# bab2min/Kiwi

Measured on AMD Instinct MI355X. Metric: sentences/sec on batched analyze(), device kernels with inputs resident in HBM (dictionary scan + lattice + Viterbi/Knlm, top-1); host-to-host rate: see e2e, higher is better.
Workload: dtype int32+f32; 1 GPU; c2-64k: 65536 synthetic sentences ({'exact_jamo': 40}), synthetic 'full' model (kiwi_amd/synth.py), Knlm, top-1; sentences_per_gpu=65536, chunks_per_gpu=65536, jamo_per_gpu=2621440, parallelism=shard1, device_bytes=9402884427, rerun_chunks=0

## Files before the change

### kiwi_amd/csrc/engine.hip

```cpp
#include <hip/hip_runtime.h>
#include <unistd.h>
#include <cstdio>
#include <cstring>
#include <ctime>
#include <algorithm>
#include <atomic>
#include <cstdlib>
#include <chrono>
#include <condition_variable>
#include <functional>
#include <map>
#include <mutex>
#include <numeric>
#include <stdexcept>
#include <thread>
#include "engine.hpp"
#include "pretok.hpp"
#include "hostpool.hpp"
#include "post_fast.hpp"
#include "viterbi_kernel.hpp"
#include "exact_math.hpp"
#include "cong_global.hpp"
#include "chr_freq.hpp"
#include "typo_lattice_kernel.hpp"
#include "typo_graph_kernel.hpp"
#include "cong_query_kernel.hpp"

namespace kamd
{
	__global__ void k_dict_scan(ModelView M, BatchView B, WorkView W, uint32_t chunkBegin, uint32_t chunkCount);
	template<int GW> __global__ void k_build_lattice(ModelView M, BatchView B, WorkView W, SearchParams P, const uint32_t* chunkList, uint32_t chunkCount, uint32_t ldsBytes);
	__global__ void k_build_lattice_big(ModelView M, BatchView B, WorkView W, SearchParams P, uint32_t chunkBegin, uint32_t chunkCount, uint32_t ldsBytes, uint32_t waveLayout);
	__global__ void k_lattice_wave(ModelView M, BatchView B, WorkView W, SearchParams P, const uint32_t* chunkList, uint32_t chunkCount, uint32_t ldsBytes, uint32_t matchRatio16, uint32_t expandMode);
	__global__ void k_expand_cands(ModelView M, BatchView B, WorkView W, uint32_t chunkBegin, uint32_t chunkCount, uint32_t transposedOrder, const uint8_t* distMask);
	__global__ void k_expand_pos(ModelView M, BatchView B, WorkView W, SearchParams P, uint32_t chunkBegin, uint32_t chunkCount, const float* nodeTypoAll, uint32_t useChr);
	__global__ void k_unk_chr(ModelView M, BatchView B, WorkView W, ChrView C, uint32_t chunkBegin, uint32_t chunkCount, uint32_t hiTok, uint32_t loTok);
	__global__ void k_unk_chr_freq(ModelView M, BatchView B, WorkView W, ChrView C, ChrFreqParams Q, float chrBias, uint32_t chunkBegin, uint32_t chunkCount, uint32_t hiTok, uint32_t loTok);

	namespace
	{
		void hipCheck(hipError_t e, const char* what)
		{
			if (e != hipSuccess) throw std::runtime_error{ std::string{ "HIP error in " } + what + ": " + hipGetErrorString(e) };
		}
#define HIPCHECK(x) hipCheck((x), #x)

		struct DevBlockCache
		{
			struct Block { void* p; size_t cap; int device; };
			std::mutex mu; std::vector<Block> blocks; size_t bytes = 0;
			static constexpr size_t kMaxBlocks = 256, kMaxBytes = 64ull << 30;
			static void release(const Block& b) { if (b.device < 0) (void)hipHostFree(b.p); else (void)hipFree(b.p); }
			void* take(size_t n, size_t& capOut, int device)
			{
				std::lock_guard<std::mutex> g{ mu };
				size_t best = blocks.size();
				for (size_t i = 0; i < blocks.size(); ++i)
					if (blocks[i].device == device && blocks[i].cap >= n && blocks[i].cap <= 2 * n + (1u << 20) && (best == blocks.size() || blocks[i].cap < blocks[best].cap)) best = i;
				if (best == blocks.size()) return nullptr;
// ... 258 lines not shown
		impl->device = device;
		HIPCHECK(hipSetDevice(device));
		HIPCHECK(hipStreamCreateWithFlags(&impl->stream, hipStreamNonBlocking));
		HIPCHECK(hipStreamCreateWithFlags(&impl->stream2, hipStreamNonBlocking));
		for (auto& ls : impl->latStream) HIPCHECK(hipStreamCreateWithFlags(&ls, hipStreamNonBlocking));
		{
			int least = 0, greatest = 0;
			const bool plain = [] { const char* e = std::getenv("KAMD_COPY_PRIORITY"); return !(e && std::atoi(e) == 1); }();
			if (plain || hipDeviceGetStreamPriorityRange(&least, &greatest) != hipSuccess || least == greatest) HIPCHECK(hipStreamCreateWithFlags(&impl->streamCopy, hipStreamNonBlocking));
			else HIPCHECK(hipStreamCreateWithPriority(&impl->streamCopy, hipStreamNonBlocking, greatest));
		}
		HIPCHECK(hipEventCreateWithFlags(&impl->lastDone, hipEventDisableTiming)); HIPCHECK(hipEventCreateWithFlags(&impl->joinEv, hipEventDisableTiming));
		HIPCHECK(hipEventCreate(&impl->latFork)); for (auto& ev : impl->latJoin) HIPCHECK(hipEventCreate(&ev));

		if (const char* sb = std::getenv("KAMD_SUBBATCHES")) impl->subBatches = std::atoi(sb);
		const FlatModel& m = impl->model;
		ModelView& v = impl->dview;
		v.h = m.h;
		using I_ = Engine::Impl;
		v.forms = impl->up(m.forms, I_::kTempForms); v.formChars = impl->up(m.formChars, I_::kTempChars); v.formCand = impl->up(m.formCand, I_::kTempCand);
		{
			std::vector<MorphRec> dm = m.morphs;
			for (size_t i = 0; i < dm.size(); ++i) { dm[i].feat = (uint16_t)m.morphPath[i]; dm[i].prevFlags = (uint8_t)(m.morphPath[i] >> 16); }
			v.morphs = impl->up(dm, I_::kTempMorphs);
			std::vector<CandStatic> unk(2);
			for (int k = 0; k < 2; ++k)
			{
				const uint32_t mid = (k == 0 ? T_NNG : T_NNP) + 1u;
				std::memcpy(&unk[k].m0, &dm[mid], 32);
				const uint32_t firstWid = (dm[mid].flags & MF_SINGLE) ? dm[mid].lmId : m.chunkLm[dm[mid].chunkOff];
				unk[k].x = Quad{ mid, firstWid, 0, 0 };
			}
			v.unkPacks = impl->up(unk);
		}
		v.chunkMorph = impl->up(m.chunkMorph, I_::kTempChunks); v.chunkLm = impl->up(m.chunkLm, I_::kTempChunks); v.chunkPos = impl->up(m.chunkPos, 2 * I_::kTempChunks);
		v.sbInfo = impl->up(m.sbInfo, I_::kTempMorphs); v.morphPath = impl->up(m.morphPath, I_::kTempMorphs);
		v.trie = impl->up(m.trie); v.trieKeys = impl->up(m.trieKeys); v.trieChild = impl->up(m.trieChild); v.trieRoot = impl->up(m.trieRoot);
		v.trieEdges = impl->up(m.trieEdges); v.trieEdgeMask = m.trieEdgeMask;
		v.lmNodes = impl->up(m.lmNodes); v.lmKeys = impl->up(m.lmKeys); v.lmValues = impl->up(m.lmValues); v.lmRoot = impl->up(m.lmRoot);
		if (m.congDim)
		{
			v.lmHash = impl->up(m.congHash); v.lmHashMask = m.congHashMask; v.lmRoot2 = impl->up(m.congRoot2); v.lmBackoff = impl->up(m.congBackoff);
			v.h.bosNode = 0;
			impl->cong = CongDev{ impl->up(m.congCtxEmb), impl->up(m.congOutEmb), m.congDim, m.congDim + 8, m.congVlTMax, m.congVlBits };
			impl->hasCong = true;
			if (impl->wantCongGlobal)
			{
				if (!m.congWindow) throw std::runtime_error{ "Cannot open ConG model with distant tokens: the file has no window sections" };
				if (m.congWindow != 7) throw std::runtime_error{ "kiwi_amd: CoNgram window size must be 7 (the reference instantiates CoNgramState<7> only)" };
				CongGDev& g = impl->congG;
				g.ctxConf = impl->up(m.congCtxConf); g.distEmb = impl->up(m.congDistEmb); g.distConf = impl->up(m.congDistConf); g.posConf = impl->up(m.congPosConf);
				g.distMask = impl->up(m.congDistMask); g.window = m.congWindow; g.keyBytes = m.congKeyBytes; g.hist = nullptr; g.itemScratch = nullptr;
				impl->hasCongG = true;
			}
		}
		else { v.lmHash = impl->up(m.lmHash); v.lmHashMask = m.lmHashMask; v.lmRoot2 = impl->up(m.lmRoot2); v.lmBackoff = impl->up(m.lmBackoff); }
		v.lmHtxNode = (m.congDim || m.lmHtxNode.empty()) ? nullptr : impl->up(m.lmHtxNode);
		v.formDialect = nullptr;
		v.morphDialect = m.morphDialect.empty() ? nullptr : impl->up(m.morphDialect, I_::kTempMorphs);
		if (v.morphDialect) HIPCHECK(hipMemset(const_cast<uint16_t*>(v.morphDialect) + m.morphDialect.size(), 0, 2 * I_::kTempMorphs));
		v.formUnkChr = nullptr; v.formChrTok = nullptr;
		v.lmChain = nullptr;
		if (!m.congDim && !m.lmBackoff.empty())
		{
			std::vector<uint32_t> chain(2 * m.lmBackoff.size());
			for (size_t n = 0; n < m.lmBackoff.size(); ++n)
// ... 525 lines not shown
			b.order = order;
			b.subBatches = S;
			if (b.typo.typo)
			{
				b.typoOrder.resize(nC);
				std::iota(b.typoOrder.begin(), b.typoOrder.end(), 0u);
				for (uint32_t k = 0; k < S; ++k)
				{
					const uint32_t c0 = (uint32_t)((uint64_t)nC * k / S), c1 = (uint32_t)((uint64_t)nC * (k + 1) / S);
					std::stable_sort(b.typoOrder.begin() + c0, b.typoOrder.begin() + c1, [&](uint32_t a, uint32_t c) { return b.typoNeed[a] > b.typoNeed[c]; });
				}
				upload(b.dTypoOrder, b.typoOrder, I.streamCopy);
			}
			HIPCHECK(hipStreamSynchronize(I.streamCopy));
		}
		const size_t nEv = 6 * (size_t)S + 2;
		while (I.evs.size() < nEv) { hipEvent_t e; HIPCHECK(hipEventCreate(&e)); I.evs.push_back(e); }
		if (I.haveLast) HIPCHECK(hipStreamWaitEvent(sA, I.lastDone, 0));
		if (b.pretok && b.pretok->hasTemps())
		{
			const TempOverlay& o = b.pretok->overlay; const FlatModel& m = I.model; const ModelView& v = I.dview;
			using I_ = Engine::Impl;
			if (o.forms.size() > I_::kTempForms || o.morphs.size() > I_::kTempMorphs || o.formChars.size() > I_::kTempChars || o.formCand.size() > I_::kTempCand || o.chunkMorph.size() > I_::kTempChunks)
				throw std::invalid_argument{ "kiwi_amd: too many temporary forms / morphemes in the pretokenized spans of one call" };
			auto put = [&](const auto* devBase, size_t at, const auto& vec)
			{
				using T = std::remove_cv_t<std::remove_pointer_t<decltype(devBase)>>;
				if (!vec.empty()) HIPCHECK(hipMemcpyAsync(const_cast<T*>(devBase) + at, vec.data(), vec.size() * sizeof(T), hipMemcpyHostToDevice, sA));
			};
			put(v.forms, o.nBaseForms, o.forms); put(v.formChars, m.formChars.size() - 1, o.formChars); put(v.formCand, m.formCand.size(), o.formCand);
			put(v.morphs, o.nBaseMorphs, b.pretok->devMorphs); put(v.chunkMorph, m.chunkMorph.size(), o.chunkMorph); put(v.chunkLm, m.chunkLm.size(), o.chunkLm);
			put(v.chunkPos, m.chunkPos.size(), o.chunkPos); put(v.sbInfo, o.nBaseMorphs, o.sbInfo); put(v.morphPath, o.nBaseMorphs, o.morphPath);
			if (v.formUnkChr) { put(v.formUnkChr, o.nBaseForms, o.formUnkChr); put(v.formChrTok, m.formChars.size() - 1, o.formChrTok); }
		}
		HIPCHECK(hipMemsetAsync(b.dResults.p, 0, nC * sizeof(DevChunkResult), sA));
		HIPCHECK(hipMemsetAsync(b.dOutCounters.p, 0, 128, sA));
		HIPCHECK(hipMemcpyAsync(b.dStateAt.p, b.wv.stateBase, (size_t)nC * 8, hipMemcpyDeviceToDevice, sA));
		if (b.slotCap) HIPCHECK(hipMemsetAsync(b.dSlotTable.p, 0, (size_t)I.histSlots() * 16, sA));
		HIPCHECK(hipMemsetAsync(I.counter.p, 0, 256, sA));
		HIPCHECK(hipMemsetAsync(b.dNNodes.p, 0, (size_t)nC * 4, sA));
		HIPCHECK(hipMemsetAsync(b.dExpanded.p, 0, nC, sA));
		if (getenv("KAMD_HANGDUMP")) HIPCHECK(hipMemsetAsync(b.dNodeStCnt.p, 0xFF, (size_t)b.nodeBase[nC] * 4, sA));
		const bool variant64 = I.histStates() ? !(I.groupLanesForced && I.groupLanes == 16) : (I.groupLanesForced && I.groupLanes == 64);
		const uint32_t nGroups = (I.histStates() || b.typo.typo || I.hasCong) ? (variant64 ? 1u : 4u)
			: 64u / (uint32_t)(I.groupLanesForced ? I.groupLanes : 8);
		const uint32_t maxWork = (nC + S - 1) / S + 1;
		const uint32_t persistBlocks = I.histStates() ? I.persistBlocks / 12 * I.histBlocksPerCu() : I.persistBlocks;
		const uint32_t maxBlocks = std::min(persistBlocks, (maxWork + nGroups - 1) / nGroups);
		const size_t groupScratchBytes = I.hasSbg ? sizeof(GroupScratchT<BIGQ_SBG>) : I.hasCongG ? sizeof(GroupScratchCong<BIGQ_SBG>) : I.hasCong ? sizeof(GroupScratchCong<BIGQ>) : sizeof(GroupScratch);
		I.bigScratch.ensure((size_t)maxBlocks * nGroups * groupScratchBytes * std::min(S, 2u));
		b.wv.bigScratch = I.bigScratch.as<uint8_t>(); b.wv.bigScratchBytes = (uint32_t)groupScratchBytes;
		if (I.histStates())
		{
			const void* before = I.sbgScratch.p;
			I.sbgScratch.ensure((size_t)maxBlocks * nGroups * sizeof(SbgScratch) * std::min(S, 2u));
			if (I.sbgScratch.p != before) HIPCHECK(hipMemsetAsync(I.sbgScratch.p, 0, I.sbgScratch.cap, sA));
		}
		const uint32_t ldsBytes = searchKernelLdsBytes(I.groupLanes);
		if (!b.typo.typo)
		{
			const bool wave = I.latticeWave && I.latticeGroupForced == 0;
			const uint32_t ratioKey = wave ? (I.latticeRatio16 & 0x3FFFu) : 0x10000u;
			const uint32_t budget = b.pretok ? 0u : wave ? I.latticeWaveBudget : I.latticeLdsBudget;
			const uint32_t classesKey = ratioKey * 31u + budget / 16u;
			if (b.latClassesKey != classesKey || b.latClasses.size() != S)
			{
// ... 1491 lines not shown
```

### kiwi_amd/csrc/flat_model.hpp

```cpp
#pragma once
#include <cstdint>
#include <cmath>
#include <string>
#include <vector>
#include "kchars.hpp"

namespace kamd
{
	enum FormFlag : uint8_t
	{
		FF_ZCODA_APPENDABLE = 1, FF_ZSIOT_APPENDABLE = 2, FF_HAS_JCLASS = 4, FF_HAS_ANY_FULL = 8,
		FF_FIRST_IS_CODA = 16,
		FF_IS_STAG = 32,
		FF_STARTS_WITH_A = 64,
		FF_ENDS_WITH_SSC = 128,
	};
	struct FormRec
	{
		uint32_t candOff;
		uint32_t charOff;
		uint16_t candCnt;
		uint8_t len;
		uint8_t numSpaces;
		uint8_t flags;
// ... 49 lines not shown
	struct TrieEdgeSlot { uint32_t node, key, child; int32_t value; };
	static_assert(sizeof(TrieEdgeSlot) == 16, "TrieEdgeSlot");
	constexpr uint32_t TRIE_EDGE_EMPTY = 0xFFFFFFFFu;
	KAMD_HD uint32_t trieEdgeHash(uint32_t node, uint32_t key) { uint32_t h = node * 0x9E3779B1u + key * 0x85EBCA6Bu; h ^= h >> 15; h *= 0x2C1B3C6Du; h ^= h >> 13; return h; }
	constexpr int32_t TRIE_NONE = -1, TRIE_SUBMATCH = -2;
	constexpr uint16_t LF_STR_SSC = 1u << 13, LF_PREV_ZSIOT = 1u << 14, LF_TAG_SSC = 1u << 15;

	struct LmSlot { uint32_t node, wid; int32_t value; float ll; };
	static_assert(sizeof(LmSlot) == 16, "LmSlot");
	constexpr uint32_t LM_SLOT_EMPTY = 0xFFFFFFFFu;
	struct LmRootRec { int32_t value; float ll; };
	struct LmBackoff { int32_t lower; float gamma; };
	KAMD_HD uint32_t lmHashOf(uint32_t node, uint32_t wid) { uint32_t h = node * 0x9E3779B1u ^ (wid * 0x85EBCA77u); h ^= h >> 15; h *= 0x2C1B3C6Du; h ^= h >> 13; return h; }

	struct LmNodeRec
	{
		uint32_t nextOff, numNexts;
		int32_t lower;
		float ll, gamma;
	};
	static_assert(sizeof(LmNodeRec) == 20, "LmNodeRec");

	struct ModelHeader
	{
		uint32_t nForms, nMorphs, vocabSize, nTrieNodes, nTrieEdges, nLmNodes, nLmEdges;
		int32_t bosNode;
		float unkLl;
		uint32_t specialMorph[6];
		uint32_t maxFormLen;
		uint32_t lmOrder;
		uint32_t lmKeyBytes;
	};

	struct ModelView
	{
		ModelHeader h;
		const FormRec* forms;
		const uint16_t* formChars;
		const uint32_t* formCand;
		const MorphRec* morphs;
		const uint32_t* chunkMorph;
		const uint32_t* chunkLm;
		const uint8_t* chunkPos;
		const uint8_t* sbInfo;
		const uint32_t* morphPath;
		const TrieNodeRec* trie;
		const uint16_t* trieKeys;
		const uint32_t* trieChild;
		const uint32_t* trieRoot;
		const LmNodeRec* lmNodes;
		const uint32_t* lmKeys;
		const int32_t* lmValues;
		const int32_t* lmRoot;
		const LmSlot* lmHash; uint32_t lmHashMask;
		const LmRootRec* lmRoot2;
		const LmBackoff* lmBackoff;
		const void* unkPacks;
		const int32_t* lmHtxNode;
		const float* formUnkChr;
		const uint16_t* formChrTok;
		const uint16_t* formDialect; const uint16_t* morphDialect;
		const uint32_t* lmChain;
		const TrieEdgeSlot* trieEdges; uint32_t trieEdgeMask;
	};

	struct SbgView
	{
		uint32_t vocabSize = 0, windowSize = 0;
		const uint32_t* ptrs = nullptr;
		const uint32_t* keys = nullptr;
		const float* comps = nullptr;
		const float* discnts = nullptr;
		const uint8_t* valid = nullptr;
		float logWindowSize = 0;
		bool present() const { return vocabSize != 0; }
	};

	struct CongNodeRec { uint32_t nextOff, numNexts; int32_t lower; uint32_t value; };
	struct CongView
	{
		uint32_t dim = 0, stride = 0, nCtx = 0, vocabSize = 0;
		const uint8_t* ctxEmb = nullptr; const uint8_t* outEmb = nullptr;
		const CongNodeRec* nodes = nullptr; const uint32_t* keys = nullptr; const int32_t* values = nullptr; const int32_t* root = nullptr;
		uint32_t rootSize = 0;
		uint32_t vlTMax = 0xFFFFFFFFu, vlBits = 0;
		uint32_t window = 0;
		uint32_t keyBytes = 4;
		const float* ctxConf = nullptr;
		const uint8_t* distEmb = nullptr;
		const float* distConf = nullptr;
// ... 276 lines not shown
```

### kiwi_amd/csrc/lattice_expand.hpp

```cpp
#pragma once
#include <hip/hip_runtime.h>
#include "device_types.hpp"
#include "feature.hpp"

namespace kamd
{
	__device__ __forceinline__ float leftBoundaryScore(uint32_t t)
	{
		if (t == 2 * T_MAX) return 5.f;
		if (t < T_MAX) return (t == T_NNP || t == T_NP || t == T_IC) ? -1.f : (t == T_SB ? -3.f : 0.f);
		const uint8_t r = (uint8_t)(t - T_MAX);
		return (isEClass(r) || isJClass(r) || isSuffixTag(r) || r == T_VCP) ? -1.f : 0.f;
	}
	__device__ __forceinline__ uint32_t posCandKind(const SearchParams& P, uint32_t flags, uint8_t tag, bool spaceBefore)
	{
		if (P.splitComplex && (flags & MF_HAS_COMPLEX)) return 0;
		if (tag == T_Z_CODA || tag == T_Z_SIOT) return (tag == T_Z_SIOT && !(P.splitSaisiot || P.mergeSaisiot)) ? 0u : 2u;
		if (!(flags & MF_SINGLE) && (flags & MF_HA_CONTRACTION) && spaceBefore) return 0;
		return 1;
	}

	__device__ __forceinline__ CandStatic candStaticOf(const ModelView& M, uint32_t mid)
	{
		const uint4* mr = reinterpret_cast<const uint4*>(M.morphs + mid);
		CandStatic o; const uint4 r0 = mr[0], r1 = mr[1];
		o.m0 = Quad{ r0.x, r0.y, r0.z, r0.w }; o.m1 = Quad{ r1.x, r1.y, r1.z, r1.w };
		const uint32_t flags = o.m1.y & 0xFFFF; const uint8_t tag = (uint8_t)o.m1.z;
		const uint32_t firstWid = (flags & MF_SINGLE) ? o.m0.x : M.chunkLm[o.m0.z];
		const uint32_t sbType = tag == T_SB ? M.sbInfo[mid] : 0;
		const uint32_t secondWid = (!(flags & MF_SINGLE) && (o.m1.w & 0xFF) >= 2) ? M.chunkLm[o.m0.z + 1] : 0;
		o.x = Quad{ mid, firstWid, sbType, secondWid };
		return o;
	}
	__device__ __forceinline__ uint32_t candClassOf(uint32_t tag, uint32_t socket, uint32_t flags)
	{
		if (tag == T_Z_CODA) return 0;
		if (tag == T_Z_SIOT) return 1;
		if (!socket) return 2;
		return (flags & MF_SINGLE) ? 3 : 4;
	}
}
```

### kiwi_amd/csrc/lattice_kernels.hip

```cpp
#include <hip/hip_runtime.h>
#include "device_types.hpp"
#include "feature.hpp"
#include "lattice_connect.hpp"
#include "lattice_expand.hpp"
#include "chr_freq.hpp"

namespace kamd
{
	__device__ __forceinline__ uint32_t trieChild(const ModelView& M, uint32_t node, uint16_t c, int32_t& value)
	{
		if (node == 0) { const uint32_t ch = M.trieRoot[c]; value = ch ? M.trie[ch].value : TRIE_NONE; return ch; }
		uint32_t h = trieEdgeHash(node, c) & M.trieEdgeMask;
		for (;;)
		{
			const uint4 s = reinterpret_cast<const uint4*>(M.trieEdges)[h];
			if (s.x == node && s.y == (uint32_t)c) { value = (int32_t)s.w; return s.z; }
			if (s.x == TRIE_EDGE_EMPTY) { value = TRIE_NONE; return 0; }
			h = (h + 1) & M.trieEdgeMask;
		}
	}

	__global__ void __launch_bounds__(256) k_dict_scan(ModelView M, BatchView B, WorkView W, uint32_t chunkBegin, uint32_t chunkCount)
	{
		const uint32_t lane = threadIdx.x & 63;
// ... 719 lines not shown
		DevNode* fin = W.nodes + nBase;
		const uint32_t textOff = B.textOffset[chunk];
		for (uint32_t idx = 0; idx < G; ++idx) latticeEmitNode(M, L, str, cls, queue, fin, idx, n, nConn, textOff);
		{
			uint32_t packTop = 0;
			const uint32_t packCap = W.packBase[chunk + 1] - W.packBase[chunk];
			for (uint32_t i = 0; i < nConn; ++i) { fin[i].packOff = packTop; packTop += fin[i].candCnt; }
			if (packTop > packCap) { W.results[chunk].status = CS_ERR_NODE_OVERFLOW; return; }
		}
		W.nNodes[chunk] = nConn;
		if (nConn <= 2) W.results[chunk].status = CS_NO_LATTICE;
	}

	__global__ void __launch_bounds__(64) k_expand_cands(ModelView M, BatchView B, WorkView W, uint32_t chunkBegin, uint32_t chunkCount, uint32_t transposedOrder, const uint8_t* distMask)
	{
		if (blockIdx.x >= chunkCount) return;
		const uint32_t chunk = chunkBegin + blockIdx.x;
		if (W.results[chunk].status != CS_OK || W.expanded[chunk]) return;
		const uint32_t nBase = W.nodeBase[chunk], G = W.nNodes[chunk];
		CandStatic* packs = W.packs + W.packBase[chunk];
		const uint32_t* blk = W.blockBits;
		auto blocked = [&](uint32_t m2) -> bool { return blk && ((blk[m2 >> 5] >> (m2 & 31)) & 1); };
		for (uint32_t i = 1 + threadIdx.x; i + 1 < G; i += blockDim.x)
		{
			const DevNode nd = W.nodes[nBase + i];
			if (nd.form == NOFORM) continue;
			const uint32_t candOff = M.forms[nd.form].candOff;
			uint32_t kept = 0;
			for (uint32_t k = 0; k < nd.candCnt; ++k)
			{
				const uint32_t mid = M.formCand[candOff + k];
				if (blocked(mid)) continue;
				++kept;
				const CandStatic o = candStaticOf(M, mid);
				uint32_t at = 0;
				if (transposedOrder)
				{
					auto cls = [&](uint32_t m2) -> uint32_t
					{
						const MorphRec r = M.morphs[m2];
						uint32_t c2 = 2u * candClassOf(r.tag, r.socket, r.flags);
						if (distMask && c2 == 4u) { const uint32_t fw = (r.flags & MF_SINGLE) ? r.lmId : M.chunkLm[r.chunkOff]; c2 += (distMask[fw >> 3] >> (fw & 7)) & 1u; }
						return c2;
					};
					const uint32_t mine = cls(mid);
					for (uint32_t j = 0; j < nd.candCnt; ++j)
					{
						if (j == k) continue;
						const uint32_t mj = M.formCand[candOff + j];
						if (blocked(mj)) continue;
						const uint32_t other = cls(mj);
						if (other < mine || (other == mine && j < k)) ++at;
					}
				}
				else if (blk) { for (uint32_t j = 0; j < k; ++j) if (!blocked(M.formCand[candOff + j])) ++at; }
				else at = k;
				packs[nd.packOff + at] = o;
			}
			if (kept != nd.candCnt) W.nodes[nBase + i].candCnt = (uint16_t)kept;
		}
	}

	__global__ void __launch_bounds__(64) k_expand_pos(ModelView M, BatchView B, WorkView W, SearchParams P, uint32_t chunkBegin, uint32_t chunkCount, const float* nodeTypoAll, uint32_t useChr)
	{
		if (blockIdx.x >= chunkCount) return;
		const uint32_t lane = threadIdx.x;
		const uint32_t chunk = chunkBegin + blockIdx.x;
// ... 257 lines not shown
```

### kiwi_amd/csrc/lattice_wave.hip

```cpp
#include <hip/hip_runtime.h>
#include "device_types.hpp"
#include "feature.hpp"
#include "lattice_expand.hpp"

namespace kamd
{
	extern __shared__ __align__(16) uint8_t lSmem[];

	namespace lw
	{
		enum OpFlag : uint16_t
		{
			OF_HASUNK = 1, OF_CONDBU = 2,
			OF_LIMJ = 4, OF_HASAPP = 8, OF_SEOK = 16, OF_QUAL = 32, OF_ZBITS = 64 | 128, OF_VALID = 256, OF_ZSEL = 512 | 1024, OF_END = 2048,
		};
		constexpr uint32_t kMaxRounds = 16;

		__device__ __forceinline__ uint32_t topBit(uint64_t m) { return 63u - (uint32_t)__builtin_clzll(m); }
		__device__ __forceinline__ uint32_t trimmedLen(const uint16_t* str, uint32_t off, uint32_t len)
		{
			while (len && isSpace(str[off + len - 1])) --len;
			return len;
		}
	}
// ... 657 lines not shown
			if (s4 && keep[nb]) { uint32_t r = base[nb] + cntA[nb] + ((ds >> 8) & 0xFFu); for (uint32_t i = 0; i < 4; ++i) if ((s4 >> i) & 1) cc[r++] = 0; }
			if ((dt & 1u) && keep[e])
			{
				const uint32_t src = opSrc[T];
				uint32_t fc = 0;
				if (!(src & 0x8000u)) fc = mfc[src];
				else { const uint32_t form = miscForm[src & 0x7FFFu]; if (form != NOFORM) fc = factsOf(form); miscFc[src & 0x7FFFu] = fc; }
				cc[base[e] + ((dt >> 1) & 0x7FFFu)] = fc & 0x7FFFu;
			}
		}
		waveSync();
		LW_MARK(11)
		uint32_t packTop = 0;
		for (uint32_t b0 = 0; b0 < nConn; b0 += 64)
		{
			const uint32_t i = b0 + lane;
			const uint32_t c = i < nConn ? cc[i] : 0u;
			uint32_t incl = c;
			for (uint32_t d = 1; d < 64; d <<= 1) { const uint32_t v = __shfl_up(incl, d); if (lane >= d) incl += v; }
			if (i < nConn) cc[i] = packTop + incl - c;
			packTop += __shfl(incl, 63);
		}
		waveSync();
		if (packTop > W.packBase[chunk + 1] - W.packBase[chunk])
		{
			if (lane == 0) W.results[chunk].status = CS_ERR_NODE_OVERFLOW;
			return;
		}
		const bool doExpand = (expandMode & 1u) != 0, transposed = (expandMode & 2u) != 0;
		const uint32_t G = nConn;
		const uint32_t nUniq = B.spOff[chunk + 1] - B.spOff[chunk];
		CandStatic* packs = W.packs + W.packBase[chunk];
		const CandStatic* unkPacks = reinterpret_cast<const CandStatic*>(M.unkPacks);
		PosRec* recs = doExpand ? W.posRecs + W.packBase[chunk] : nullptr;
		PosDesc* desc = doExpand ? W.posDesc + nBase : nullptr;
		uint32_t* posSlow = grpOff; uint32_t* posPass1 = posA; uint32_t* posIdx = posZ;
		bool posOk = doExpand && G > 2 && G <= 0xFFF0u && nUniq + 1 <= 0x1Fu;
		uint32_t nPos = 0, recTop = 0;
		auto spaceBeforeOf = [&](uint32_t s0, bool isEnd) -> bool
		{
			const uint32_t startStr = isEnd ? n : (uint32_t)nsToPos[s0];
			return s0 == 0 ? (textOff + startStr > 0) : ((uint32_t)nsToPos[s0 - 1] + 1u < startStr);
		};
		if (doExpand)
		{
			if (lane == 0) { desc[0].firstNode = 0; desc[0].nNodes = 0; desc[0].flags = 0; desc[0].firstRec = 0; desc[0].nRec = 0; }
			for (uint32_t q = lane; q < nPosAll; q += 64) { posSlow[q] = 0; posPass1[q] = 0; }
			if (lane == 0) recOff[0] = 0;
			waveSync();
			for (uint32_t T = 1 + lane; T <= K; T += 64)
			{
				const uint32_t ne = opNE[T], nb = ne & 0xFFFF, e = ne >> 16, fl = opFl[T], ds = decS[T], s4 = ds & 15u, dt = decT[T];
				if (s4 && keep[nb])
				{
					uint32_t r = base[nb] + cntA[nb] + ((ds >> 8) & 0xFFu);
					for (uint32_t i = 0; i < 4; ++i) if ((s4 >> i) & 1) recOff[r++] = 2;
					const uint32_t bu = opBU[T];
					uint32_t lp = dt >> 16;
					if ((s4 & 5u) && lp && isHangulCoda(str[nsToPos[lp]])) --lp;
					for (uint32_t i = 0; i < 4; ++i)
					{
						if (!((s4 >> i) & 1)) continue;
						const uint32_t s0 = (i & 1) ? ((i & 2) ? (bu >> 16) : (bu & 0xFFFF)) : lp;
						if (s0 && cntA[s0] + cntU[s0] > 256) atomicOr(&posSlow[nb], 1u);
					}
				}
				if ((dt & 1u) && keep[e])
				{
					const uint32_t rank = (dt >> 1) & 0x7FFFu, src = opSrc[T], ni = base[e] + rank;
					if (fl & OF_END) { recOff[ni] = 0; continue; }
					uint32_t form, fc;
					if (src & 0x8000u) { form = miscForm[src & 0x7FFFu]; fc = miscFc[src & 0x7FFFu]; } else { form = mforms[src]; fc = mfc[src]; }
					if (nb && cntA[nb] + cntU[nb] > 256) atomicOr(&posSlow[e], 1u);
					if (form == NOFORM) { recOff[ni] = 2; continue; }
					const uint32_t candCnt = fc & 0x7FFFu, candOff = M.forms[form].candOff, pk = cc[ni];
					const bool spaceBefore = spaceBeforeOf(nb, false);
					uint32_t cnt = 0, classCnt[5] = { 0, 0, 0, 0, 0 };
					if (transposed)
						for (uint32_t k = 0; k < candCnt; ++k) { const MorphRec r = M.morphs[M.formCand[candOff + k]]; ++classCnt[candClassOf(r.tag, r.socket, r.flags)]; }
					uint32_t classAt[5] = { 0, classCnt[0], classCnt[0] + classCnt[1], classCnt[0] + classCnt[1] + classCnt[2], classCnt[0] + classCnt[1] + classCnt[2] + classCnt[3] };
					for (uint32_t k = 0; k < candCnt; ++k)
					{
						const CandStatic o = candStaticOf(M, M.formCand[candOff + k]);
						const uint32_t flags = o.m1.y & 0xFFFF; const uint8_t tag = (uint8_t)o.m1.z;
						const uint32_t at = transposed ? classAt[candClassOf(tag, o.m1.z >> 24, flags)]++ : k;
						packs[pk + at] = o;
						if (posCandKind(P, flags, tag, spaceBefore)) ++cnt;
					}
					if (cnt == 0) atomicOr(&posSlow[e], 1u);
					if ((fc & 0x8000u) && rank < 16) atomicOr(&posPass1[e], 1u << rank);
					recOff[ni] = cnt + ((fc & 0x8000u) ? 1u : 0u);
				}
			}
			waveSync();
			for (uint32_t b0 = 0; b0 < G; b0 += 64)
			{
				const uint32_t i = b0 + lane;
				const uint32_t c = i < G ? recOff[i] : 0u;
				uint32_t incl = c;
				for (uint32_t d = 1; d < 64; d <<= 1) { const uint32_t v = __shfl_up(incl, d); if (lane >= d) incl += v; }
				if (i < G) recOff[i] = recTop + incl - c;
				recTop += __shfl(incl, 63);
			}
			for (uint32_t b0 = 0; b0 < nPosAll; b0 += 64)
			{
				const uint32_t q = b0 + lane;
				const bool has = q >= 1 && q <= nNs && keep[q] && cntA[q] + cntU[q] > 0;
				const uint64_t hb = __ballot(has);
				if (q < nPosAll) posIdx[q] = has ? nPos + 1u + (uint32_t)__popcll(hb & ((1ull << lane) - 1ull)) : 0u;
				nPos += (uint32_t)__popcll(hb);
			}
			const uint32_t recCap = W.packBase[chunk + 1] - W.packBase[chunk];
			if (recTop > recCap || recTop >= 0x3FFFFu || nPos >= 0x1FFFu) posOk = false;
			waveSync();
			if (posOk)
			{
				uint32_t* posMask = W.posMask + nBase;
				bool overAny = false;
				for (uint32_t q = 1 + lane; q <= nNs; q += 64)
				{
// ... 2 lines not shown
					const uint32_t n0 = base[q], nN = cntA[q] + cntU[q], r0 = recOff[n0], r1 = n0 + nN < G ? recOff[n0 + nN] : recTop;
					const bool slow = nN > 16 || r1 - r0 > 16 || r1 == r0 || posSlow[q] != 0;
					uint32_t st4[4] = { 0, 0, 0, 0 }, nSt = 0; bool over = nPos > 255;
					for (uint64_t m = pred[q]; m && !over; m &= m - 1)
					{
						const uint32_t len = (uint32_t)__ffsll((unsigned long long)m), sp = posIdx[q - len];
						if (nSt == 4) { over = true; break; }
						st4[nSt++] = sp;
					}
					for (uint32_t t = nSt; t < 4; ++t) st4[t] = st4[0];
					posMask[p] = over ? 0xFFFFFFFFu : (st4[0] | (st4[1] << 8) | (st4[2] << 16) | (st4[3] << 24));
					overAny = overAny || over;
					const uint32_t a = cntA[q], tot = nN < 16 ? nN : 16u;
					const uint32_t formless = a < 16 ? (((1u << tot) - 1u) & ~((1u << a) - 1u)) : 0u;
					PosDesc d;
					d.firstNode = (uint16_t)n0; d.nNodes = (uint8_t)(nN > 255 ? 255 : nN); d.flags = slow ? (uint8_t)POSF_SLOW : (uint8_t)0;
					d.firstRec = r0; d.nRec = (uint16_t)(r1 - r0 > 0xFFFF ? 0xFFFF : r1 - r0); d.pad = (uint16_t)formless; d.pad2 = posPass1[q];
					desc[p] = d;
				}
				if (__ballot(overAny) && lane == 0) desc[0].nNodes = 1;
				if (lane == 0)
				{
					PosDesc d; d.firstNode = (uint16_t)(G - 1); d.nNodes = 0; d.flags = 0; d.firstRec = recTop; d.nRec = 0; d.pad = 0; d.pad2 = 0;
					desc[nPos + 1] = d;
					desc[0].pad2 = posIdx[nNs];
				}
			}
		}
		auto emitNode = [&](uint32_t ni, uint32_t s, uint32_t t, uint32_t form, uint32_t fc, uint32_t uOff, uint32_t uLen, uint32_t se, uint32_t rankAt, bool isEnd)
		{
			DevNode nn;
			nn.form = form; nn.uformOff = (uint16_t)uOff; nn.uformLen = (uint16_t)uLen; nn.spaceErrors = (uint8_t)(se > 255 ? 255 : se);
			nn.ownFeat = 0; nn.pad = 0; nn.packOff = cc[ni];
			const bool pnBos = s == 0;
			const bool spaceBefore = spaceBeforeOf(s, isEnd);
			bool lb = pnBos || spaceBefore;
			const uint32_t pu = firstU[s];
			if (!lb && (pu >> 16))
			{
				const uint32_t lp = (pu & 0xFFFF) + (pu >> 16) - 1;
				const uint16_t c = str[lp];
				const uint8_t tag = (isLowSurrogate(c) || isHighSurrogate(c)) ? (uint8_t)T_SH : (uint8_t)(cls[lp] & 0x3F);
				if (tag == T_SSC || c == u'"' || c == u'\'') lb = false;
				else if (T_SF <= tag && tag <= T_SB) lb = true;
			}
			uint8_t nf = 0;
			if (spaceBefore) nf |= NF_SPACE_BEFORE;
			if (lb) nf |= NF_LEFT_BOUNDARY;
			if (uLen && str[uOff + uLen - 1] == u'.') nf |= NF_UFORM_ENDS_POINT;
			if (fc & 0x8000u) nf |= NF_ALL_PARTIAL;
			nn.nPrev = (uint16_t)(pnBos ? 1u : cntA[s] + cntU[s]);
			nn.candCnt = (uint16_t)(fc & 0x7FFFu); nn.fflags = (uint8_t)(fc >> 16); nn.flen = (uint8_t)(fc >> 24);
			if (uLen)
			{
				uint16_t of = featMaskFast(str + uOff, uLen) & 0x1FFF;
				const uint32_t lp = uOff + uLen - 1;
				const uint16_t c = str[lp];
				const uint8_t tag = (isLowSurrogate(c) || isHighSurrogate(c)) ? (uint8_t)T_SH : (uint8_t)(cls[lp] & 0x3F);
				if (tag == T_SSC) of |= LF_STR_SSC;
				nn.ownFeat = of;
			}
			nn.nflags = nf;
			nn.prev = (uint16_t)(ni - base[s]);
			nn.sibling = (!isEnd && rankAt + 1 < cntA[t] + cntU[t]) ? 1 : 0;
			if (isEnd) nn.startPos = nn.endPos = (uint16_t)n;
			else { nn.startPos = nsToPos[s]; nn.endPos = (uint16_t)(nsToPos[t - 1] + 1); }
			fin[ni] = nn;
			if (!posOk || isEnd) return;
			{
				const uint32_t np1 = (uint32_t)nn.nPrev - 1u, sp = posIdx[s];
				(W.posPrev + nBase)[ni] = base[s] | ((np1 > 255u ? 255u : np1) << 16) | ((sp > 255u ? 255u : sp) << 24);
			}
			const uint32_t nl = rankAt;
			if (nl >= 16) return;
			PosRec* out = recs + recOff[ni];
			float ws = 0;
			if (!nn.uformLen && nn.form != NOFORM && nn.flen && nn.spaceErrors) ws = -P.spacePenalty * (float)nn.spaceErrors;
			const float baseDiscount = ws + (-0.f * P.typoCostWeight);
			const uint8_t ownKind0 = nn.uformLen ? 1 : 0;
			auto emit = [&](const CandStatic* cs, float disc, uint8_t ownKind, uint16_t ownFeat, uint32_t extra)
			{
				const uint4* q4 = reinterpret_cast<const uint4*>(cs);
				const uint4 m0 = q4[0], m1 = q4[1], mx = q4[2];
				const uint8_t tag = (uint8_t)m1.z, special = (uint8_t)(m1.w >> 24);
				const uint32_t sbType = mx.z;
				const bool quote = special == 0 || special == 1 || special == 3 || special == 4;
				const uint32_t R = ((sbType || quote) && nUniq > 1) ? nUniq : 1u;
				PosRec r;
				r.firstWid = mx.y; r.secondWid = mx.w; r.chunkOff = m0.z; r.lastSeqId = m0.y;
				r.morph = mx.x; r.flagsFeat = m1.y; r.tagw = m1.z; r.cntw = m1.w;
				r.additional = __uint_as_float(m0.w) + disc + leftBoundaryScore(((nn.nflags & NF_LEFT_BOUNDARY) ? T_MAX : 0) + clearIrregular(tag)) * 5.f;
				const uint32_t ruleBits = ((isEClass(tag) && (nn.fflags & FF_STARTS_WITH_A)) ? 1u : 0u) | ((tag == T_SN && (nn.nflags & NF_UFORM_ENDS_POINT)) ? 2u : 0u)
					| ((M.morphDialect && M.morphDialect[r.morph]) ? 4u : 0u);
				r.nodeOwn = ni | ((uint32_t)ownFeat << 16);
				r.bits = (sbType & 0xFF) | (ruleBits << 8) | ((uint32_t)ownKind << 16) | ((uint32_t)nn.nflags << 24);
				r.rq = R | (nl << 8) | extra;
				*out++ = r;
			};
			auto sharedFirstWord = [&](const CandStatic* cl, uint32_t nc) -> uint32_t
			{
				if (!transposed) return 0u;
				uint32_t nReg = 0, ref = 0; bool one = true;
				for (uint32_t k = 0; k < nc; ++k)
				{
					const uint4* q4 = reinterpret_cast<const uint4*>(cl + k);
					const uint4 m1 = q4[1], mx = q4[2];
					const uint32_t flags = m1.y & 0xFFFF; const uint8_t tag = (uint8_t)m1.z, sock = (uint8_t)(m1.z >> 24);
					if (posCandKind(P, flags, tag, spaceBefore) != 1 || sock || (flags & MF_FIRST_WID_IS_P)) continue;
					if (!nReg) ref = mx.y; else if (mx.y != ref) one = false;
					++nReg;
				}
				return (nReg && one) ? (uint32_t)PR_OUT_FIRST : 0u;
			};
			if (nn.form != NOFORM)
			{
				const CandStatic* cl = packs + nn.packOff;
				const uint32_t of0 = sharedFirstWord(cl, nn.candCnt);
				for (uint32_t k = 0; k < nn.candCnt; ++k)
				{
					const uint4 m1 = reinterpret_cast<const uint4*>(cl + k)[1];
					const uint32_t kind = posCandKind(P, m1.y & 0xFFFF, (uint8_t)m1.z, spaceBefore);
					if (kind == 1) emit(cl + k, baseDiscount + 0.f, ownKind0, nn.ownFeat, of0);
					else if (kind == 2)
					{
						const MorphRec cm = M.morphs[reinterpret_cast<const uint4*>(cl + k)[2].x];
						const MorphRec nm = M.morphs[cm.lmId];
						PosRec r;
						r.firstWid = cm.lmId; r.secondWid = cm.tag; r.chunkOff = (uint32_t)nm.feat | ((uint32_t)nm.prevFlags << 16) | (nm.socket ? 1u << 24 : 0u); r.lastSeqId = 0;
						r.morph = cm.lmId; r.flagsFeat = 0; r.tagw = 0; r.cntw = 0;
						r.additional = cm.userScore;
						r.nodeOwn = ni; r.bits = (uint32_t)nn.nflags << 24; r.rq = 1u | (nl << 8) | (uint32_t)PR_Z;
						*out++ = r;
					}
				}
				if (nn.nflags & NF_ALL_PARTIAL)
				{
					const FormRec f = M.forms[nn.form];
					uint16_t of = featMaskFast(M.formChars + f.charOff, f.len) & 0x1FFF;
					if (f.flags & FF_ENDS_WITH_SSC) of |= LF_STR_SSC;
					const float disc = baseDiscount + -((float)f.len * P.oovRuleScale + P.oovRuleBias);
					emit(unkPacks + 1, disc, 2, of, (uint32_t)PR_PASS1 | sharedFirstWord(unkPacks + 1, 1));
				}
			}
			else
			{
				const float emo = (cls[nn.uformOff] & 0x80) ? -10.f : 0.f;
				const float disc = baseDiscount + (emo - ((float)nn.uformLen * P.oovRuleScale + P.oovRuleBias));
				const uint32_t of0 = sharedFirstWord(unkPacks, 2);
				emit(unkPacks, disc, ownKind0, nn.ownFeat, of0);
				emit(unkPacks + 1, disc, ownKind0, nn.ownFeat, of0);
			}
		};
		if (lane == 0)
		{
			DevNode bos; bos.form = NOFORM; bos.startPos = bos.endPos = 0; bos.prev = bos.sibling = 0; bos.uformOff = bos.uformLen = 0; bos.spaceErrors = 0; bos.nflags = 0; bos.nPrev = 0; bos.packOff = 0; bos.candCnt = 0; bos.fflags = 0; bos.flen = 0; bos.ownFeat = 0; bos.pad = 0;
			fin[0] = bos;
		}
		for (uint32_t T = 1 + lane; T <= K; T += 64)
		{
			const uint32_t ne = opNE[T], nb = ne & 0xFFFF, e = ne >> 16, fl = opFl[T], s4 = decS[T] & 15u, dt = decT[T];
			if (s4 && keep[nb])
			{
				const uint32_t bu = opBU[T];
				uint32_t lp = dt >> 16;
				if ((s4 & 5u) && lp && isHangulCoda(str[nsToPos[lp]])) --lp;
				uint32_t r = cntA[nb] + ((decS[T] >> 8) & 0xFFu);
				for (uint32_t i = 0; i < 4; ++i)
				{
					if (!((s4 >> i) & 1)) continue;
					const uint32_t s0 = (i & 1) ? ((i & 2) ? (bu >> 16) : (bu & 0xFFFF)) : lp;
					const uint32_t o = nsToPos[s0], len = nsToPos[nb - 1] + 1u - o, l = plain ? len : trimmedLen(str, o, len);
					emitNode(base[nb] + r, s0, nb, NOFORM, 0, o, l, 0, r, false);
					++r;
				}
			}
			if ((dt & 1u) && keep[e])
			{
				const uint32_t rank = (dt >> 1) & 0x7FFFu, src = opSrc[T];
				uint32_t form, fc, uOff = 0, uLen = 0, se = 0;
				if (src & 0x8000u) { form = miscForm[src & 0x7FFFu]; fc = miscFc[src & 0x7FFFu]; const uint32_t mu = miscU[src & 0x7FFFu]; uOff = mu & 0xFFFF; uLen = mu >> 16; }
				else { form = mforms[src]; fc = mfc[src]; se = mse[src]; }
				emitNode(base[e] + rank, nb, e, form, fc, uOff, uLen, se, rank, (fl & OF_END) != 0);
			}
// ... 16 lines not shown
```

### kiwi_amd/csrc/pretok.cpp

```cpp
#include <algorithm>
#include <stdexcept>
#include "pretok.hpp"
#include "textprep.hpp"
#include "kchars.hpp"

namespace kamd
{
	namespace
	{
		inline bool tagsEqual(uint8_t a, uint8_t b, bool infer) { return infer ? ((a & 0x7F) == (b & 0x7F)) : (a == b); }
		inline uint32_t defaultMorphemeId(uint8_t tag) { return (uint32_t)(tag & 0x7F) + 1u; }
	}

	void makePretokGroup(const FlatModel& m, const char16_t* text, size_t len, uint64_t match, const std::vector<PtSpan>& spans, PretokGroup& g)
	{
		g = PretokGroup{};
		if (spans.empty()) return;
		U16 norm; std::vector<uint32_t> pos;
		normalizeWithPosition(text, len, norm, pos);
		if (match & M_NORMALIZE_CODA) normalizeCoda(norm);
		const uint32_t nM = m.h.nMorphs, nF = m.h.nForms;
		TempEntries& temps = g.temps;
		for (const PtSpan& sp : spans)
		{
			if (sp.begin >= sp.end || sp.end > len) throw std::invalid_argument{ "pretokenized span outside the text or empty" };
			const uint32_t b = pos[sp.begin], e = pos[sp.end];
			if (b >= e) throw std::invalid_argument{ "pretokenized span outside the text or empty" };
			PretokGroup::Span sn{ b, e, 0, false };
			if (sp.tokens.empty())
			{
				const int32_t f = formIdOfString(m, norm.substr(b, e - b));
				sn.form = f >= 0 ? (uint32_t)f : (uint32_t)T_NNP - 1u;
			}
			else if (sp.tokens.size() == 1)
			{
				const PtToken& t = sp.tokens[0];
				U16 fs; std::vector<uint32_t> dp;
// ... 33 lines not shown
					uint32_t found = 0xFFFFFFFFu;
					if (f >= 0)
						for (uint32_t ci = 0; ci < m.forms[f].candCnt; ++ci)
						{
							const uint32_t mi = m.formCand[m.forms[f].candOff + ci];
							if (m.morphs[mi].tag == t.tag) { found = mi; break; }
						}
					if (found == 0xFFFFFFFFu)
					{
						found = nM + (uint32_t)temps.morphs.size();
						temps.morphs.push_back(TempEntries::Morph{ (uint32_t)temps.forms.size(), t.tag, defaultMorphemeId(t.tag), {} });
						temps.forms.push_back(TempEntries::Form{ fs, {} });
					}
					if (t.begin > t.end || (uint64_t)sp.begin + t.end > len) throw std::invalid_argument{ "token range outside its pretokenized span's text" };
					const uint32_t cb = pos[sp.begin + t.begin] - b, ce = pos[sp.begin + t.end] - b;
					if (cb > 255 || ce > 255) throw std::invalid_argument{ "pretokenized span longer than 255 units" };
					chunks.push_back(TempEntries::Chunk{ found, (uint8_t)cb, (uint8_t)ce });
				}
				temps.morphs[wholeAt].chunks = std::move(chunks);
				sn.form = nF + wholeForm;
			}
			sn.fallback = sn.form + 1 >= (uint32_t)T_NNG && sn.form + 1 < (uint32_t)T_MAX;
			g.spans.push_back(sn);
		}
		std::stable_sort(g.spans.begin(), g.spans.end(), [](const PretokGroup::Span& a, const PretokGroup::Span& c) { return a.begin < c.begin; });
		for (size_t i = 1; i < g.spans.size(); ++i)
			if (g.spans[i - 1].end > g.spans[i].begin) throw std::invalid_argument{ "`PretokenizedSpan`s should not have overlapped ranges." };
		if (!temps.forms.empty())
		{
			bakeTempsOverlay(m, temps, g.overlay);
			const TempOverlay& o = g.overlay;
			g.devMorphs = o.morphs;
			for (size_t i = 0; i < g.devMorphs.size(); ++i) { g.devMorphs[i].feat = (uint16_t)o.morphPath[i]; g.devMorphs[i].prevFlags = (uint8_t)(o.morphPath[i] >> 16); }
			FlatModel& hm = g.hostModel;
			hm.h = m.h; hm.h.nForms = nF + (uint32_t)temps.forms.size(); hm.h.nMorphs = nM + (uint32_t)temps.morphs.size();
			hm.morphs = m.morphs; hm.morphs.insert(hm.morphs.end(), o.morphs.begin(), o.morphs.end());
			hm.morphKform = m.morphKform; hm.morphKform.insert(hm.morphKform.end(), o.morphKform.begin(), o.morphKform.end());
			hm.forms.assign(m.forms.begin(), m.forms.begin() + nF); hm.forms.insert(hm.forms.end(), o.forms.begin(), o.forms.end());
			hm.formChars.assign(m.formChars.begin(), m.formChars.end() - 1); hm.formChars.insert(hm.formChars.end(), o.formChars.begin(), o.formChars.end());
			if (!m.morphDialect.empty()) { hm.morphDialect = m.morphDialect; hm.morphDialect.resize(hm.morphs.size(), 0); }
		}
	}
}
```

### kiwi_amd/csrc/pretok.hpp

```cpp
#pragma once
#include <cstdint>
#include <string>
#include <vector>
#include "flat_model.hpp"

namespace kamd
{
	struct PtToken { std::u16string form; uint32_t begin, end; uint8_t tag; bool inferRegularity; };
	struct PtSpan { uint32_t begin, end; std::vector<PtToken> tokens; };
	struct PretokGroup
	{
		struct Span { uint32_t begin, end, form; bool fallback; };
		std::vector<Span> spans;
		TempEntries temps;
		TempOverlay overlay;
		std::vector<MorphRec> devMorphs;
		FlatModel hostModel;
		bool hasTemps() const { return !overlay.empty(); }
	};
	void makePretokGroup(const FlatModel& m, const char16_t* text, size_t len, uint64_t match, const std::vector<PtSpan>& spans, PretokGroup& out);
}
```

Before: 14.92 million sentences/s.

## Precompute per-candidate static packs on host and read them directly in lattice kernels

Builds a CandStatic table per formCand entry once at model load, plus a class-transposed copy when a CoNgram model is present, and uploads both, with pretokenized overlays patched in per call. Lattice kernels then copy contiguous precomputed packs instead of gathering morph records and chunkLm/sbInfo through indirection, and the emit path reads candidates straight from the table. This removes dependent global loads and per-candidate class counting, at the cost of extra device memory (48 bytes per candidate, doubled for ConG) and more host setup work.

Result: no change. 15.03 million sentences/s (median of 6 runs) (+0.7%).

```diff
diff --git a/kiwi_amd/csrc/engine.hip b/kiwi_amd/csrc/engine.hip
--- a/kiwi_amd/csrc/engine.hip
+++ b/kiwi_amd/csrc/engine.hip
@@ -25,6 +25,7 @@
 #include "typo_lattice_kernel.hpp"
 #include "typo_graph_kernel.hpp"
 #include "cong_query_kernel.hpp"
+#include "lattice_expand.hpp"
 
 namespace kamd
 {
@@ -349,6 +350,24 @@
 				unk[k].x = Quad{ mid, firstWid, 0, 0 };
 			}
 			v.unkPacks = impl->up(unk);
+			std::vector<CandStatic> cs(m.formCand.size());
+			for (size_t i = 0; i < cs.size(); ++i)
+			{
+				const uint32_t mid = m.formCand[i];
+				if (mid >= dm.size()) { cs[i] = CandStatic{}; continue; }
+				cs[i] = candStaticOf(dm[mid], mid, [&](uint32_t c) -> uint32_t { return c < m.chunkLm.size() ? m.chunkLm[c] : 0u; }, [&]() -> uint32_t { return mid < m.sbInfo.size() ? m.sbInfo[mid] : 0u; });
+			}
+			v.candStatic = impl->up(cs, I_::kTempCand);
+			if (m.congDim)
+			{
+				std::vector<CandStatic> ct = cs;
+				for (uint32_t f = 0; f < m.h.nForms; ++f)
+				{
+					const size_t at = m.forms[f].candOff, cnt = m.forms[f].candCnt & 0x7FFFu;
+					if (at + cnt <= cs.size()) candStaticTransposed(cs.data() + at, (uint32_t)cnt, ct.data() + at);
+				}
+				v.candStaticT = impl->up(ct, I_::kTempCand);
+			}
 		}
 		v.chunkMorph = impl->up(m.chunkMorph, I_::kTempChunks); v.chunkLm = impl->up(m.chunkLm, I_::kTempChunks); v.chunkPos = impl->up(m.chunkPos, 2 * I_::kTempChunks);
 		v.sbInfo = impl->up(m.sbInfo, I_::kTempMorphs); v.morphPath = impl->up(m.morphPath, I_::kTempMorphs);
@@ -940,6 +959,8 @@
 			put(v.morphs, o.nBaseMorphs, b.pretok->devMorphs); put(v.chunkMorph, m.chunkMorph.size(), o.chunkMorph); put(v.chunkLm, m.chunkLm.size(), o.chunkLm);
 			put(v.chunkPos, m.chunkPos.size(), o.chunkPos); put(v.sbInfo, o.nBaseMorphs, o.sbInfo); put(v.morphPath, o.nBaseMorphs, o.morphPath);
 			if (v.formUnkChr) { put(v.formUnkChr, o.nBaseForms, o.formUnkChr); put(v.formChrTok, m.formChars.size() - 1, o.formChrTok); }
+			put(v.candStatic, m.formCand.size(), b.pretok->devCand);
+			if (v.candStaticT) put(v.candStaticT, m.formCand.size(), b.pretok->devCandT);
 		}
 		HIPCHECK(hipMemsetAsync(b.dResults.p, 0, nC * sizeof(DevChunkResult), sA));
 		HIPCHECK(hipMemsetAsync(b.dOutCounters.p, 0, 128, sA));
diff --git a/kiwi_amd/csrc/flat_model.hpp b/kiwi_amd/csrc/flat_model.hpp
--- a/kiwi_amd/csrc/flat_model.hpp
+++ b/kiwi_amd/csrc/flat_model.hpp
@@ -105,6 +105,7 @@
 		uint32_t lmKeyBytes;
 	};
 
+	struct CandStatic;
 	struct ModelView
 	{
 		ModelHeader h;
@@ -129,6 +130,7 @@
 		const LmRootRec* lmRoot2;
 		const LmBackoff* lmBackoff;
 		const void* unkPacks;
+		const CandStatic* candStatic = nullptr; const CandStatic* candStaticT = nullptr;
 		const int32_t* lmHtxNode;
 		const float* formUnkChr;
 		const uint16_t* formChrTok;
diff --git a/kiwi_amd/csrc/lattice_expand.hpp b/kiwi_amd/csrc/lattice_expand.hpp
--- a/kiwi_amd/csrc/lattice_expand.hpp
+++ b/kiwi_amd/csrc/lattice_expand.hpp
@@ -20,23 +20,29 @@
 		return 1;
 	}
 
-	__device__ __forceinline__ CandStatic candStaticOf(const ModelView& M, uint32_t mid)
+	template<class ChunkLm, class SbInfo> inline CandStatic candStaticOf(const MorphRec& r, uint32_t mid, ChunkLm&& chunkLm, SbInfo&& sbInfo)
 	{
-		const uint4* mr = reinterpret_cast<const uint4*>(M.morphs + mid);
-		CandStatic o; const uint4 r0 = mr[0], r1 = mr[1];
-		o.m0 = Quad{ r0.x, r0.y, r0.z, r0.w }; o.m1 = Quad{ r1.x, r1.y, r1.z, r1.w };
+		static_assert(sizeof(MorphRec) == 2 * sizeof(Quad), "MorphRec");
+		CandStatic o;
+		__builtin_memcpy(&o.m0, &r, sizeof(Quad)); __builtin_memcpy(&o.m1, reinterpret_cast<const char*>(&r) + sizeof(Quad), sizeof(Quad));
 		const uint32_t flags = o.m1.y & 0xFFFF; const uint8_t tag = (uint8_t)o.m1.z;
-		const uint32_t firstWid = (flags & MF_SINGLE) ? o.m0.x : M.chunkLm[o.m0.z];
-		const uint32_t sbType = tag == T_SB ? M.sbInfo[mid] : 0;
-		const uint32_t secondWid = (!(flags & MF_SINGLE) && (o.m1.w & 0xFF) >= 2) ? M.chunkLm[o.m0.z + 1] : 0;
+		const uint32_t firstWid = (flags & MF_SINGLE) ? o.m0.x : chunkLm(o.m0.z);
+		const uint32_t sbType = tag == T_SB ? sbInfo() : 0;
+		const uint32_t secondWid = (!(flags & MF_SINGLE) && (o.m1.w & 0xFF) >= 2) ? chunkLm(o.m0.z + 1) : 0;
 		o.x = Quad{ mid, firstWid, sbType, secondWid };
 		return o;
 	}
-	__device__ __forceinline__ uint32_t candClassOf(uint32_t tag, uint32_t socket, uint32_t flags)
+	KAMD_HD uint32_t candClassOf(uint32_t tag, uint32_t socket, uint32_t flags)
 	{
 		if (tag == T_Z_CODA) return 0;
 		if (tag == T_Z_SIOT) return 1;
 		if (!socket) return 2;
 		return (flags & MF_SINGLE) ? 3 : 4;
 	}
+	inline uint32_t candClassOf(const CandStatic& c) { return candClassOf(c.m1.z & 0xFF, c.m1.z >> 24, c.m1.y & 0xFFFF); }
+	inline void candStaticTransposed(const CandStatic* in, uint32_t cnt, CandStatic* out)
+	{
+		uint32_t at = 0;
+		for (uint32_t c = 0; c < 5; ++c) for (uint32_t k = 0; k < cnt; ++k) if (candClassOf(in[k]) == c) out[at++] = in[k];
+	}
 }
diff --git a/kiwi_amd/csrc/lattice_kernels.hip b/kiwi_amd/csrc/lattice_kernels.hip
--- a/kiwi_amd/csrc/lattice_kernels.hip
+++ b/kiwi_amd/csrc/lattice_kernels.hip
@@ -775,7 +775,7 @@
 				const uint32_t mid = M.formCand[candOff + k];
 				if (blocked(mid)) continue;
 				++kept;
-				const CandStatic o = candStaticOf(M, mid);
+				const CandStatic o = M.candStatic[candOff + k];
 				uint32_t at = 0;
 				if (transposedOrder)
 				{
diff --git a/kiwi_amd/csrc/lattice_wave.hip b/kiwi_amd/csrc/lattice_wave.hip
--- a/kiwi_amd/csrc/lattice_wave.hip
+++ b/kiwi_amd/csrc/lattice_wave.hip
@@ -713,6 +713,7 @@
 		const uint32_t nUniq = B.spOff[chunk + 1] - B.spOff[chunk];
 		CandStatic* packs = W.packs + W.packBase[chunk];
 		const CandStatic* unkPacks = reinterpret_cast<const CandStatic*>(M.unkPacks);
+		const CandStatic* candTab = transposed ? M.candStaticT : M.candStatic;
 		PosRec* recs = doExpand ? W.posRecs + W.packBase[chunk] : nullptr;
 		PosDesc* desc = doExpand ? W.posDesc + nBase : nullptr;
 		uint32_t* posSlow = grpOff; uint32_t* posPass1 = posA; uint32_t* posIdx = posZ;
@@ -754,19 +755,21 @@
 					if (src & 0x8000u) { form = miscForm[src & 0x7FFFu]; fc = miscFc[src & 0x7FFFu]; } else { form = mforms[src]; fc = mfc[src]; }
 					if (nb && cntA[nb] + cntU[nb] > 256) atomicOr(&posSlow[e], 1u);
 					if (form == NOFORM) { recOff[ni] = 2; continue; }
-					const uint32_t candCnt = fc & 0x7FFFu, candOff = M.forms[form].candOff, pk = cc[ni];
+					const uint32_t candCnt = fc & 0x7FFFu, pk = cc[ni];
+					const CandStatic* tab = candTab + M.forms[form].candOff;
 					const bool spaceBefore = spaceBeforeOf(nb, false);
-					uint32_t cnt = 0, classCnt[5] = { 0, 0, 0, 0, 0 };
-					if (transposed)
-						for (uint32_t k = 0; k < candCnt; ++k) { const MorphRec r = M.morphs[M.formCand[candOff + k]]; ++classCnt[candClassOf(r.tag, r.socket, r.flags)]; }
-					uint32_t classAt[5] = { 0, classCnt[0], classCnt[0] + classCnt[1], classCnt[0] + classCnt[1] + classCnt[2], classCnt[0] + classCnt[1] + classCnt[2] + classCnt[3] };
-					for (uint32_t k = 0; k < candCnt; ++k)
-					{
-						const CandStatic o = candStaticOf(M, M.formCand[candOff + k]);
-						const uint32_t flags = o.m1.y & 0xFFFF; const uint8_t tag = (uint8_t)o.m1.z;
-						const uint32_t at = transposed ? classAt[candClassOf(tag, o.m1.z >> 24, flags)]++ : k;
-						packs[pk + at] = o;
-						if (posCandKind(P, flags, tag, spaceBefore)) ++cnt;
+					uint32_t cnt = 0;
+					for (uint32_t k = 0; k < candCnt; k += 4)
+					{
+						uint2 ft[4];
+						for (uint32_t j = 0; j < 4; ++j) { const uint32_t kj = k + j < candCnt ? k + j : candCnt - 1; ft[j] = *reinterpret_cast<const uint2*>(reinterpret_cast<const uint32_t*>(tab + kj) + 5); }
+						for (uint32_t j = 0; j < 4; ++j) if (k + j < candCnt && posCandKind(P, ft[j].x & 0xFFFF, (uint8_t)ft[j].y, spaceBefore)) ++cnt;
+					}
+					{
+						const uint4* src = reinterpret_cast<const uint4*>(tab); uint4* dst = reinterpret_cast<uint4*>(packs + pk);
+						const uint32_t nq = 3u * candCnt;
+						uint32_t q = 0;
+						for (; q < nq; q += 3) { const uint4 a = src[q], b = src[q + 1], c = src[q + 2]; dst[q] = a; dst[q + 1] = b; dst[q + 2] = c; }
 					}
 					if (cnt == 0) atomicOr(&posSlow[e], 1u);
 					if ((fc & 0x8000u) && rank < 16) atomicOr(&posPass1[e], 1u << rank);
@@ -835,6 +838,7 @@
 			DevNode nn;
 			nn.form = form; nn.uformOff = (uint16_t)uOff; nn.uformLen = (uint16_t)uLen; nn.spaceErrors = (uint8_t)(se > 255 ? 255 : se);
 			nn.ownFeat = 0; nn.pad = 0; nn.packOff = cc[ni];
+			const uint32_t candOff = (posOk && !isEnd && form != NOFORM) ? M.forms[form].candOff : 0u;
 			const bool pnBos = s == 0;
 			const bool spaceBefore = spaceBeforeOf(s, isEnd);
 			bool lb = pnBos || spaceBefore;
@@ -881,10 +885,9 @@
 			if (!nn.uformLen && nn.form != NOFORM && nn.flen && nn.spaceErrors) ws = -P.spacePenalty * (float)nn.spaceErrors;
 			const float baseDiscount = ws + (-0.f * P.typoCostWeight);
 			const uint8_t ownKind0 = nn.uformLen ? 1 : 0;
-			auto emit = [&](const CandStatic* cs, float disc, uint8_t ownKind, uint16_t ownFeat, uint32_t extra)
-			{
-				const uint4* q4 = reinterpret_cast<const uint4*>(cs);
-				const uint4 m0 = q4[0], m1 = q4[1], mx = q4[2];
+			const uint4* unkQ = reinterpret_cast<const uint4*>(unkPacks);
+			auto emit = [&](const uint4 m0, const uint4 m1, const uint4 mx, float disc, uint8_t ownKind, uint16_t ownFeat, uint32_t extra)
+			{
 				const uint8_t tag = (uint8_t)m1.z, special = (uint8_t)(m1.w >> 24);
 				const uint32_t sbType = mx.z;
 				const bool quote = special == 0 || special == 1 || special == 3 || special == 4;
@@ -917,21 +920,22 @@
 			};
 			if (nn.form != NOFORM)
 			{
-				const CandStatic* cl = packs + nn.packOff;
+				const CandStatic* cl = candTab + candOff;
 				const uint32_t of0 = sharedFirstWord(cl, nn.candCnt);
 				for (uint32_t k = 0; k < nn.candCnt; ++k)
 				{
-					const uint4 m1 = reinterpret_cast<const uint4*>(cl + k)[1];
+					const uint4* q4 = reinterpret_cast<const uint4*>(cl + k);
+					const uint4 m0 = q4[0], m1 = q4[1], mx = q4[2];
 					const uint32_t kind = posCandKind(P, m1.y & 0xFFFF, (uint8_t)m1.z, spaceBefore);
-					if (kind == 1) emit(cl + k, baseDiscount + 0.f, ownKind0, nn.ownFeat, of0);
+					if (kind == 1) emit(m0, m1, mx, baseDiscount + 0.f, ownKind0, nn.ownFeat, of0);
 					else if (kind == 2)
 					{
-						const MorphRec cm = M.morphs[reinterpret_cast<const uint4*>(cl + k)[2].x];
-						const MorphRec nm = M.morphs[cm.lmId];
+						const uint32_t lmId = m0.x;
+						const MorphRec nm = M.morphs[lmId];
 						PosRec r;
-						r.firstWid = cm.lmId; r.secondWid = cm.tag; r.chunkOff = (uint32_t)nm.feat | ((uint32_t)nm.prevFlags << 16) | (nm.socket ? 1u << 24 : 0u); r.lastSeqId = 0;
-						r.morph = cm.lmId; r.flagsFeat = 0; r.tagw = 0; r.cntw = 0;
-						r.additional = cm.userScore;
+						r.firstWid = lmId; r.secondWid = m1.z & 0xFFu; r.chunkOff = (uint32_t)nm.feat | ((uint32_t)nm.prevFlags << 16) | (nm.socket ? 1u << 24 : 0u); r.lastSeqId = 0;
+						r.morph = lmId; r.flagsFeat = 0; r.tagw = 0; r.cntw = 0;
+						r.additional = __uint_as_float(m0.w);
 						r.nodeOwn = ni; r.bits = (uint32_t)nn.nflags << 24; r.rq = 1u | (nl << 8) | (uint32_t)PR_Z;
 						*out++ = r;
 					}
@@ -942,7 +946,7 @@
 					uint16_t of = featMaskFast(M.formChars + f.charOff, f.len) & 0x1FFF;
 					if (f.flags & FF_ENDS_WITH_SSC) of |= LF_STR_SSC;
 					const float disc = baseDiscount + -((float)f.len * P.oovRuleScale + P.oovRuleBias);
-					emit(unkPacks + 1, disc, 2, of, (uint32_t)PR_PASS1 | sharedFirstWord(unkPacks + 1, 1));
+					emit(unkQ[3], unkQ[4], unkQ[5], disc, 2, of, (uint32_t)PR_PASS1 | sharedFirstWord(unkPacks + 1, 1));
 				}
 			}
 			else
@@ -950,8 +954,8 @@
 				const float emo = (cls[nn.uformOff] & 0x80) ? -10.f : 0.f;
 				const float disc = baseDiscount + (emo - ((float)nn.uformLen * P.oovRuleScale + P.oovRuleBias));
 				const uint32_t of0 = sharedFirstWord(unkPacks, 2);
-				emit(unkPacks, disc, ownKind0, nn.ownFeat, of0);
-				emit(unkPacks + 1, disc, ownKind0, nn.ownFeat, of0);
+				emit(unkQ[0], unkQ[1], unkQ[2], disc, ownKind0, nn.ownFeat, of0);
+				emit(unkQ[3], unkQ[4], unkQ[5], disc, ownKind0, nn.ownFeat, of0);
 			}
 		};
 		if (lane == 0)
diff --git a/kiwi_amd/csrc/pretok.cpp b/kiwi_amd/csrc/pretok.cpp
--- a/kiwi_amd/csrc/pretok.cpp
+++ b/kiwi_amd/csrc/pretok.cpp
@@ -3,6 +3,7 @@
 #include "pretok.hpp"
 #include "textprep.hpp"
 #include "kchars.hpp"
+#include "lattice_expand.hpp"
 
 namespace kamd
 {
@@ -102,6 +103,22 @@
 			const TempOverlay& o = g.overlay;
 			g.devMorphs = o.morphs;
 			for (size_t i = 0; i < g.devMorphs.size(); ++i) { g.devMorphs[i].feat = (uint16_t)o.morphPath[i]; g.devMorphs[i].prevFlags = (uint8_t)(o.morphPath[i] >> 16); }
+			g.devCand.resize(o.formCand.size());
+			for (size_t i = 0; i < o.formCand.size(); ++i)
+			{
+				const uint32_t mid = o.formCand[i];
+				MorphRec r;
+				if (mid < nM) { r = m.morphs[mid]; r.feat = (uint16_t)m.morphPath[mid]; r.prevFlags = (uint8_t)(m.morphPath[mid] >> 16); }
+				else r = g.devMorphs[mid - nM];
+				g.devCand[i] = candStaticOf(r, mid, [&](uint32_t c) { return c < m.chunkLm.size() ? m.chunkLm[c] : o.chunkLm[c - m.chunkLm.size()]; },
+					[&]() -> uint32_t { return mid < nM ? m.sbInfo[mid] : o.sbInfo[mid - nM]; });
+			}
+			g.devCandT = g.devCand;
+			for (const FormRec& f : o.forms)
+			{
+				const size_t at = f.candOff - m.formCand.size(), cnt = f.candCnt & 0x7FFFu;
+				if (f.candOff >= m.formCand.size() && at + cnt <= g.devCand.size()) candStaticTransposed(g.devCand.data() + at, (uint32_t)cnt, g.devCandT.data() + at);
+			}
 			FlatModel& hm = g.hostModel;
 			hm.h = m.h; hm.h.nForms = nF + (uint32_t)temps.forms.size(); hm.h.nMorphs = nM + (uint32_t)temps.morphs.size();
 			hm.morphs = m.morphs; hm.morphs.insert(hm.morphs.end(), o.morphs.begin(), o.morphs.end());
diff --git a/kiwi_amd/csrc/pretok.hpp b/kiwi_amd/csrc/pretok.hpp
--- a/kiwi_amd/csrc/pretok.hpp
+++ b/kiwi_amd/csrc/pretok.hpp
@@ -2,7 +2,7 @@
 #include <cstdint>
 #include <string>
 #include <vector>
-#include "flat_model.hpp"
+#include "device_types.hpp"
 
 namespace kamd
 {
@@ -15,6 +15,7 @@
 		TempEntries temps;
 		TempOverlay overlay;
 		std::vector<MorphRec> devMorphs;
+		std::vector<CandStatic> devCand, devCandT;
 		FlatModel hostModel;
 		bool hasTemps() const { return !overlay.empty(); }
 	};
```
